# julius-sk/spgemm-gnn

Measured on AMD Instinct MI355X. Metric: SpGEMM+SSpMM edges/sec on Reddit, hidden=256, k in {8,16,32,64}; %HBM roofline, higher is better.
Workload: dtype f32

## Files before the change

spgemm-gnn_amd/csrc/common.h:

```cpp
#pragma once

#include <hip/hip_runtime.h>
#include <stdint.h>

#include <string>
#include <vector>

#include "device_buf.h"
#include "maxk_hip.h"

namespace maxk {

constexpr int kWave = 64;
constexpr int kFwdTileRows = 32;
constexpr int kFwdMaxTileRows = 64;
constexpr int kFwdRowPad = 1;
constexpr int kFwdColBits = 26;
constexpr uint32_t kFwdColMask = (1u << kFwdColBits) - 1;
constexpr int kFwdThreads = 256;
constexpr int kBwdThreads = 512;
constexpr int kMaxDim = 256;
constexpr int kFwdUnroll = 8;
constexpr int kFwdFlagChunk3 = 1;
constexpr int kFwdFlagQuad = 2;
constexpr int kFwdFlagChunk2 = 4;
constexpr int kBwdTasksPerCu = 2;
constexpr int kBwdMinTaskEdges = 100000;
constexpr int kXcds = 8;
constexpr int kFwdRotWindows = 16;
constexpr double kFwdSlotEdgeRate = 1.6e8;
constexpr double kFwdSlotEdgeRateFixed = 3.0e8;
constexpr double kFwdPackedTableBytes = 150e6;
constexpr double kFwdPackedTableBytes16 = 32e6;
constexpr long long kFwdPackMinEdgesPerCol = 40;
constexpr long long kFwdPackMinEdgesPerColL2 = 128;
constexpr double kFwdSelL2Bytes = 3e6;
constexpr double kBwdTwoPassReuse = 0.75;
constexpr int kBwdRowsPerWave = 4;
constexpr double kBwdTwoPassWorkspaceCap = 16.0 * (1ull << 30);
constexpr int kStatsBlocksPerCu = 4;
constexpr int kBwdRecPad = 16 * kWave + kWave;
constexpr int kBwdLdsBudget = 160 * 1024;

void set_error(const std::string& msg);

#define MAXK_CHECK_ARG(cond, msg)                 \
  do {                                            \
    if (!(cond)) {                                \
      ::maxk::set_error(msg);                     \
      return MAXK_ERR_INVALID_ARG;                \
    }                                             \
  } while (0)

#define MAXK_HIP_TRY(expr)                                                      \
  do {                                                                          \
    hipError_t _e = (expr);                                                     \
    if (_e != hipSuccess) {                                                     \
      ::maxk::set_error(std::string(#expr) + ": " + hipGetErrorString(_e));     \
      return (int)_e;                                                           \
    }                                                                           \
  } while (0)

#define MAXK_LAUNCH_CHECK(what)                                                 \
  do {                                                                          \
    hipError_t _e = hipGetLastError();                                          \
    if (_e != hipSuccess) {                                                     \
      ::maxk::set_error(std::string(what) + ": " + hipGetErrorString(_e));      \
      return (int)_e;                                                           \
    }                                                                           \
  } while (0)

inline bool ranges_overlap(const void* a, int64_t na, const void* b, int64_t nb) {
  const uintptr_t x = reinterpret_cast<uintptr_t>(a), y = reinterpret_cast<uintptr_t>(b);
  return na > 0 && nb > 0 && x < y + (uintptr_t)nb && y < x + (uintptr_t)na;
}

struct FwdTask {
  int32_t row0;
  int32_t nrows;
  int32_t e0;
  int32_t e1;
};
static_assert(sizeof(FwdTask) == 16, "FwdTask is loaded as one dwordx4");

inline int cbsr_record_bytes(int k) {
  const int b = 5 * k;
  return b <= 64 ? 64 : b <= 128 ? 128 : (b + 15) / 16 * 16;
}

// ... 21 lines not shown
struct BwdTask {
  int32_t col0;
  int32_t ncols;
  int32_t e0;
  int32_t e1;
  int32_t shared;
  int32_t group;
  int32_t chunk;
  int32_t slab;
};
static_assert(sizeof(BwdTask) == 32, "BwdTask is 2 x dwordx4");


__device__ __forceinline__ void lds_add(double* p, double v) {
  __hip_atomic_fetch_add(p, v, __ATOMIC_RELAXED, __HIP_MEMORY_SCOPE_WORKGROUP);
}

__device__ __forceinline__ void global_add(float* p, float v) {
  __hip_atomic_fetch_add(p, v, __ATOMIC_RELAXED, __HIP_MEMORY_SCOPE_AGENT);
}

}

struct maxk_plan {
  int32_t num_nodes = 0;
  int32_t num_cols = 0;
  int64_t num_edges = 0;
  int32_t dim_origin = 0;
  int32_t dim_k = 0;
  const int32_t* src_ptr = nullptr;
  const int32_t* src_idx = nullptr;
  int32_t cus = 256;
  int32_t fwd_tile_rows = 32;
  int32_t fwd_waves = 4;
  int32_t fwd_unroll = 8;
  int32_t fwd_rec_bytes = 0;
  maxk::DeviceBuf<uint8_t> fwd_rec;
  int32_t fwd_fixed = 0;
  maxk::DeviceBuf<int2> fwd_fix;
  maxk::DeviceBuf<int32_t> fwd_rowptr;
  int64_t fwd_xstat_off = 0;
  maxk::DeviceBuf<maxk::FwdTask> fwd_tasks;
  int32_t fwd_phases = 1;
  int32_t fwd_rot_ticks = 0;
  int32_t fwd_chunk3 = 0;
  int32_t fwd_chunk2 = 0;
  int32_t fwd_quad = 0;
  int32_t fwd_two_tables = 0;
  maxk::DeviceBuf<int32_t> fwd_phase_off;
  maxk::DeviceBuf<int32_t> fwd_perm;
  maxk::DeviceBuf<uint2> fwd_cv;
  int32_t fwd_rowconst = 0;
  int32_t fwd_rowconst_off = 0;
  maxk::DeviceBuf<uint32_t> fwd_cv4;
  maxk::DeviceBuf<float> fwd_rowval;
  int32_t n_fwd_tasks = 0;
  maxk::DeviceBuf<int32_t> zero_rows;
  int32_t n_zero_rows = 0;
  int32_t bwd_feats = 4;
  int32_t bwd_slot_groups = 1;
  int32_t bwd_kp = 0;
  int32_t bwd_ks = 0;
  int32_t bwd_unroll = 8;
  int32_t bwd_waves = 8;
  int32_t bwd_big = 0;
  int32_t bwd_block_cols = 0;
  int32_t n_bwd_blocks = 0;
  maxk::DeviceBuf<maxk::BwdTask> bwd_tasks;
  int32_t n_bwd_tasks = 0;
  int32_t n_bwd_shared = 0;
  maxk::DeviceBuf<int32_t> bwd_perm;
  maxk::DeviceBuf<uint32_t> bwd_rec;
  maxk::DeviceBuf<uint32_t> bwd_sel;
  int32_t bwd_twopass = 0;
  int32_t bwd_tp_rows = 1;
  maxk::DeviceBuf<uint32_t> bwd_erec;
  maxk::DeviceBuf<float> bwd_tbuf;
  maxk::DeviceBuf<int32_t> bwd_colptr;
  int32_t bwd_tp_chunks = 1;
  std::vector<int32_t> tp_rows;
  std::vector<int64_t> tp_edges;
  maxk::DeviceBuf<int32_t> bwd_colptr2;
  int32_t col_order = 1;
  maxk::DeviceBuf<int32_t> bwd_corder;
  int64_t bwd_slab_floats = 0;
  int64_t bwd_slab_off = 0;
  maxk::DeviceBuf<int4> bwd_combine;
  int32_t n_bwd_combine = 0;
  int64_t device_bytes = 0;
  int32_t external_ws = 0;
  int64_t fwd_ws_bytes = 0;
  int64_t bwd_ws_bytes = 0;
  int32_t bwd_row_order = 1;
  int32_t fwd_handout = 1;
  int32_t bwd_handout = 1;
};

inline bool plan_fwd_rowconst_shape(const maxk_plan* p) {
  const int k = p->dim_k;
  if (!(k % 4 == 0 || p->fwd_chunk3 || p->fwd_chunk2)) return false;
  const int Lf = p->fwd_chunk3 ? (k + 2) / 3 : p->fwd_chunk2 ? k / 2 : k / 4;
  return p->fwd_quad && Lf % 4 == 0 && p->fwd_unroll == 8 && p->fwd_fix;
}

inline int plan_fwd_layout(const maxk_plan* p) {
  if (p->fwd_chunk2) return 4;
  if (p->fwd_chunk3) return 2;
  if (p->dim_k % 4 != 0) return 3;
  return p->fwd_two_tables ? 0 : 1;
}
```

spgemm-gnn_amd/csrc/plan.hip:

```cpp
#include <hipcub/hipcub.hpp>

#include <algorithm>
#include <cmath>
#include <cstddef>
#include <cstring>
#include <memory>
#include <utility>
#include <vector>

#include "common.h"

namespace maxk {


__global__ void expand_rows_kernel(const int32_t* __restrict__ ptr, int N,
                                   int32_t* __restrict__ row_of) {
  const int lane = threadIdx.x & (kWave - 1);
  const int row = blockIdx.x * (256 / kWave) + threadIdx.x / kWave;
  if (row >= N) return;
  const int e1 = ptr[row + 1];
  for (int e = ptr[row] + lane; e < e1; e += kWave) row_of[e] = row;
}

__global__ void fwd_key_kernel(const int32_t* __restrict__ idx, const int32_t* __restrict__ row_of,
// ... 571 lines not shown
                 "maxk_plan_create: fwd_chunk3 must be 0, 1, 2 or 3");
  MAXK_CHECK_REMOVED(o.bwd_cas64 == 0 || o.bwd_cas64 == 1, "bwd_cas64 = 2");
  MAXK_CHECK_REMOVED(o.quad_loads == 0, "quad_loads");
  MAXK_CHECK_ARG(o.fwd_two_tables >= 0 && o.fwd_two_tables <= 2,
                 "maxk_plan_create: fwd_two_tables must be 0, 1 or 2");
  MAXK_CHECK_ARG(o.external_workspace == 0 || o.external_workspace == 1,
                 "maxk_plan_create: external_workspace must be 0 or 1");
  MAXK_CHECK_ARG(o.bwd_flush >= 0 && o.bwd_flush <= 2,
                 "maxk_plan_create: bwd_flush must be 0, 1 or 2");
  MAXK_CHECK_ARG(o.bwd_chunk_bounds >= 0 && o.bwd_chunk_bounds <= 3,
                 "maxk_plan_create: bwd_chunk_bounds must be 0 or 2");
  MAXK_CHECK_REMOVED(o.bwd_chunk_bounds == 0 || o.bwd_chunk_bounds == 2,
                     "bwd_chunk_bounds 1 (shared rows) / 3 (equal cost)");
  MAXK_CHECK_ARG(o.fwd_fixed >= 0 && o.fwd_fixed <= 2,
                 "maxk_plan_create: fwd_fixed must be 0, 1 or 2");
  MAXK_CHECK_ARG(o.bwd_tp_store >= 0 && o.bwd_tp_store <= 2,
                 "maxk_plan_create: bwd_tp_store must be 0 or 1");
  MAXK_CHECK_REMOVED(o.bwd_tp_store != 2, "bwd_tp_store = 2 (column-order products)");
  MAXK_CHECK_REMOVED(o.bwd_row_cost == 0, "bwd_row_cost");
  MAXK_CHECK_ARG(o.col_order >= 0 && o.col_order <= 4,
                 "maxk_plan_create: col_order must be 0, 1, 2 or 4");
  MAXK_CHECK_REMOVED(o.col_order != 3, "col_order = 3 (clustered)");
  MAXK_CHECK_ARG(o.bwd_row_order >= 0 && o.bwd_row_order <= 2,
                 "maxk_plan_create: bwd_row_order must be 0, 1 or 2");
  MAXK_CHECK_ARG(o.fwd_rowconst >= 0 && o.fwd_rowconst <= 2,
                 "maxk_plan_create: fwd_rowconst must be 0, 1 or 2");
  return MAXK_OK;
}

static int device_cus() {
  int dev = 0;
  hipDeviceProp_t prop;
  if (hipGetDevice(&dev) == hipSuccess && hipGetDeviceProperties(&prop, dev) == hipSuccess &&
      prop.multiProcessorCount > 0)
    return prop.multiProcessorCount;
  return 256;
}

namespace {

struct PlanBuild {
  const int32_t* ptr;
  const int32_t* idx;
  const float* val;
  int32_t N, NC;
  int64_t E;
  int32_t D, k;
  const maxk_plan_options& o;
  const int32_t* user_order;
  hipStream_t s;
  std::vector<int32_t> hp;
  std::unique_ptr<maxk_plan> plan;
  bool big_table = false;
  int C = 1, S = 1;
  int order_mode = 1;
  bool twopass = false;
  bool row_hash_ok = false, row_hash = false;
  int64_t ra = 1, rb = 0;
  int rbits = 1;
  int nblocks = 0;
  const int32_t* bcolpos = nullptr;
  std::vector<FwdTask> ftasks;
  std::vector<int32_t> zrows;
  std::vector<int64_t> offs;
  std::vector<BwdTask> btasks;
  int nshared = 0;
  DeviceBuf<int32_t> row_of;
  DeviceBuf<int32_t> order;
  DeviceBuf<int32_t> colpos;
  DeviceBuf<uint32_t> bkeys;
  DeviceBuf<int32_t> brow;
  DeviceBuf<int32_t> bcol;
};

}

static int hip_fail(const char* what, hipError_t e) {
  set_error(std::string("maxk_plan_create: ") + what + ": " + hipGetErrorString(e));
  return (int)e;
}
#define PLAN_TRY(expr)                                         \
  do {                                                         \
    const hipError_t _e = (expr);                              \
    if (_e != hipSuccess) return hip_fail(#expr, _e);          \
  } while (0)

static int check_args(const PlanBuild& ctx) {
  const maxk_plan_options& o = ctx.o;
  const int32_t N = ctx.N, NC = ctx.NC, D = ctx.D, k = ctx.k;
  const int64_t E = ctx.E;
  const int32_t *ptr = ctx.ptr, *idx = ctx.idx, *user_order = ctx.user_order;
  if (const int rc = check_options(o)) return rc;
  MAXK_CHECK_ARG(o.col_order != 4 || user_order != nullptr || NC == 0,
                 "maxk_plan_create: col_order 4 needs the col_order argument");
  MAXK_CHECK_ARG(NC >= 0 && (E == 0 || NC > 0), "maxk_plan_create: num_cols out of range");
  if ((uint32_t)NC > kFwdColMask + 1u) {
    set_error("maxk_plan_create: more than 2^26 source columns is not supported");
    return MAXK_ERR_UNSUPPORTED;
  }
  MAXK_CHECK_ARG(N >= 0 && E >= 0 && E < (int64_t)INT32_MAX,
                 "maxk_plan_create: sizes out of range (E must fit int32)");
  MAXK_CHECK_ARG(D >= 1 && D <= kMaxDim, "maxk_plan_create: dim_origin must be in [1, 256]");
  MAXK_CHECK_ARG(k >= 1 && k <= D, "k must be between 1 and input dimension");
  MAXK_CHECK_ARG(ptr != nullptr && (E == 0 || idx != nullptr), "maxk_plan_create: null pointer");
  return MAXK_OK;
}

static void choose_fwd_shape(PlanBuild& ctx) {
  maxk_plan* p = ctx.plan.get();
  const maxk_plan_options& o = ctx.o;
  const int32_t N = ctx.N, NC = ctx.NC, D = ctx.D, k = ctx.k;
  const int cus = p->cus;
  const int fwd_row_bytes = (D + kFwdRowPad) * 8;
  const int fwd_two_wg_rows = std::min(kFwdMaxTileRows, (kBwdLdsBudget / 2 - 256) / fwd_row_bytes);
  const bool fwd_lds_two_wg = 3 * kFwdTileRows * fwd_row_bytes > kBwdLdsBudget &&
                              (int64_t)N >= (int64_t)fwd_two_wg_rows * 10 * cus;
  p->fwd_tile_rows = o.fwd_tile_rows ? o.fwd_tile_rows
                     : fwd_lds_two_wg ? fwd_two_wg_rows : kFwdTileRows;
  const int waves_rec = o.fwd_waves ? o.fwd_waves : (k == 16 && o.fwd_unroll != 4 ? 4 : 8);
  p->fwd_chunk2 = (o.fwd_chunk3 == 3 || (o.fwd_chunk3 == 0 && k == 16)) && k % 2 == 0 &&
                  k / 2 <= kWave;
  p->fwd_waves = p->fwd_chunk2 && !o.fwd_waves ? 8 : waves_rec;
  p->fwd_unroll = o.fwd_unroll ? o.fwd_unroll : (p->fwd_waves == 8 && k == 48 ? 4 : 8);
  p->fwd_chunk3 = (o.fwd_chunk3 == 1 ||
                   ((o.fwd_chunk3 == 0 || (o.fwd_chunk3 == 3 && !p->fwd_chunk2)) && k % 16 != 0)) &&
                  (k + 2) / 3 <= kWave;
  ctx.big_table = (double)std::max(NC, 1) * 5.0 * k >
                (k >= 32 ? kFwdPackedTableBytes : kFwdPackedTableBytes16);
  p->fwd_fixed = (o.fwd_fixed == 1 || (o.fwd_fixed == 0 && k >= 16 && !ctx.big_table)) &&
                 (k % 4 == 0 || p->fwd_chunk3 || p->fwd_chunk2);
  p->fwd_quad = p->fwd_fixed;
}

static void choose_bwd_shape(PlanBuild& ctx) {
  maxk_plan* p = ctx.plan.get();
  const maxk_plan_options& o = ctx.o;
  const int32_t N = ctx.N, NC = ctx.NC, D = ctx.D, k = ctx.k;
  const int64_t E = ctx.E;
  const int lds_budget = o.bwd_lds_bytes ? o.bwd_lds_bytes : kBwdLdsBudget;
  bool two_slots = false;
  if (k == 8 && N > 0 && NC > 0) {
    const double c0 = std::min<double>(NC, (lds_budget - 16) / (5.0 * k));
    two_slots = (double)E / N * c0 / NC < 10.0;
  }
  int F = o.bwd_features_per_lane ? o.bwd_features_per_lane
                                  : (two_slots || (k % 4 == 2 && k <= 2 * kWave) ? 2 : 4);
  if (F == 2 && (k + 1) / 2 > kWave) F = 4;
  p->bwd_feats = F;
  const int kF = (k + F - 1) / F * F;
  int S = o.bwd_slot_groups ? o.bwd_slot_groups : 1;
  if (o.bwd_slot_groups == 0 && F == 4 && k >= 16 && k % 8 == 0 && N > 0 && NC > 0) {
    const double c1 = std::min<double>(NC, (lds_budget - 16) / (5.0 * k));
    if ((double)E / N * c1 / NC < 4.5) S = 2;
  }
  while (S > 1 && kF % (F * S) != 0) S >>= 1;
  if (o.bwd_features_per_lane == 0 && F == 4 && S == 2 && kF / S == 8) {
    F = 2;
    p->bwd_feats = F;
  }
  p->bwd_slot_groups = S;
  p->bwd_kp = kF;
  p->bwd_ks = kF / S;
  p->bwd_unroll = o.bwd_unroll ? o.bwd_unroll : (F == 2 ? 12 : 8);
  p->bwd_waves = o.bwd_waves ? o.bwd_waves : (k >= 32 ? 12 : 8);
  p->bwd_big = (uint64_t)N * (uint64_t)D * 4u > 0xffffffffull;
  int C = std::max(1, (lds_budget - 16) / (5 * p->bwd_ks));
  C = std::min(C, std::max(NC, 1));
  ctx.C = C;
  ctx.S = S;
}

static hipError_t need_row_of(PlanBuild& ctx) {
  if (ctx.row_of || ctx.E == 0) return hipSuccess;
  const hipError_t e = ctx.row_of.alloc((size_t)ctx.E);
  if (e != hipSuccess) return e;
  hipLaunchKernelGGL(expand_rows_kernel, dim3((ctx.N + 3) / 4), dim3(256), 0, ctx.s, ctx.ptr,
                     ctx.N, ctx.row_of);
  return hipGetLastError();
}

static int read_ptr(PlanBuild& ctx) {
  const int32_t N = ctx.N;
// ... 75 lines not shown
    PLAN_TRY(hipGetLastError());
    PLAN_TRY(sort_pairs(d_tmp, d_kin, d_kout, d_ids, p->fwd_perm, E, cbits + tbits, s));
    PLAN_TRY(plan_alloc(p, p->fwd_cv, (size_t)E + 1, true));
    PLAN_TRY(hipMemsetAsync(p->fwd_cv + E, 0, sizeof(uint2), s));
    hipLaunchKernelGGL(gather_fwd_kernel, dim3(grid_for(E, 256)), dim3(256), 0, s,
                       p->fwd_perm, ctx.idx, d_rl, ctx.val, E, p->fwd_cv, true);
    PLAN_TRY(hipGetLastError());
    PLAN_TRY(hipStreamSynchronize(s));
  }
  return MAXK_OK;
}

static int build_forward(PlanBuild& ctx) {
  maxk_plan* p = ctx.plan.get();
  const maxk_plan_options& o = ctx.o;
  std::vector<FwdTask>& ftasks = ctx.ftasks;
  std::vector<int32_t>& zrows = ctx.zrows;
  const int32_t N = ctx.N, NC = ctx.NC, k = ctx.k;
  const int64_t E = ctx.E;
  hipStream_t s = ctx.s;
  build_fwd_tasks(ctx.hp, N, p->fwd_tile_rows, o.fwd_task_cap, ftasks, zrows);
  p->n_fwd_tasks = (int32_t)ftasks.size();
  p->n_zero_rows = (int32_t)zrows.size();
  if (!ftasks.empty()) {
    const int nt = (int)ftasks.size();
    if (const int rc = sort_fwd_edges(ctx)) return rc;
    PLAN_TRY(plan_alloc(p, p->fwd_tasks, ftasks.size()));
    PLAN_TRY(upload(p->fwd_tasks, ftasks, s));
    if (p->fwd_fixed) {
      PLAN_TRY(plan_alloc(p, p->fwd_fix, ftasks.size()));
      PLAN_TRY(plan_alloc(p, p->fwd_rowptr, (size_t)N + 1));
      PLAN_TRY(hipMemcpyAsync(p->fwd_rowptr, ctx.ptr, sizeof(int32_t) * ((size_t)N + 1),
                              hipMemcpyDeviceToDevice, s));
      PLAN_TRY(fwd_fix_stats(p, p->fwd_rowptr, ctx.val, s));
    }
    int B = 1;
    p->fwd_rot_ticks = 0;
    const bool low_reuse = o.fwd_rotate == 0 && NC > 0 && (double)E / NC < 64.0;
    if (o.fwd_rotate != 2 && !low_reuse && (k % 4 == 0 || p->fwd_chunk3 || p->fwd_chunk2)) {
      const int Bd = p->fwd_fixed ? (k >= 64 ? 64 : k >= 32 ? 32 : kFwdRotWindows) : kFwdRotWindows;
      B = o.fwd_rot_windows > 0 ? std::min(o.fwd_rot_windows, 64) : Bd;
      const double rate = o.fwd_rot_rate > 0 ? o.fwd_rot_rate * 1e6
                                             : std::min(5e8, std::max(2e7, (p->fwd_fixed ? kFwdSlotEdgeRateFixed : kFwdSlotEdgeRate) * 16.0 / k));
      const double tile_ticks = (double)E / nt / rate * 1e8;
      p->fwd_rot_ticks = (int)std::max(1.0, tile_ticks / B);
    }
    B = std::max(1, std::min(B, std::max(NC, 1)));
    p->fwd_phases = B;
    PLAN_TRY(plan_alloc(p, p->fwd_phase_off, (size_t)nt * (B + 1)));
    hipLaunchKernelGGL(fwd_phase_kernel, dim3((nt * (B + 1) + 255) / 256), dim3(256), 0, s,
                       p->fwd_tasks, nt, p->fwd_cv, NC, B, p->fwd_phase_off);
    PLAN_TRY(hipGetLastError());
    p->fwd_rowconst_off = o.fwd_rowconst == 2;
    PLAN_TRY(fwd_set_values(p, p->fwd_rowptr, ctx.val, true, s));
  }
  if (!zrows.empty()) {
    PLAN_TRY(plan_alloc(p, p->zero_rows, zrows.size()));
    PLAN_TRY(upload(p->zero_rows, zrows, s));
  }
  return MAXK_OK;
}

static int layout_fwd_workspace(PlanBuild& ctx) {
  maxk_plan* p = ctx.plan.get();
  const maxk_plan_options& o = ctx.o;
  const int32_t NC = ctx.NC, k = ctx.k;
  const int64_t E = ctx.E;
  const bool big_table = ctx.big_table;
  const bool sel_l2 = (double)std::max(NC, 1) * k <= kFwdSelL2Bytes;
  const bool few_edges = E < kFwdPackMinEdgesPerCol * std::max(NC, 1) ||
                         (sel_l2 && E < kFwdPackMinEdgesPerColL2 * std::max(NC, 1));
  p->fwd_two_tables = !p->fwd_chunk3 && !p->fwd_chunk2 && k % 4 == 0 &&
                      (o.fwd_two_tables == 1 ||
                       (o.fwd_two_tables == 0 &&
                        (k >= 64 || (!big_table && (k >= 32 || few_edges)))));
  if (p->fwd_two_tables) {
  } else if ((p->fwd_chunk3 || p->fwd_chunk2) && NC > 0) {
    const int b = (p->fwd_chunk3 ? (k + 2) / 3 : k / 2) * 16;
    p->fwd_rec_bytes = b <= 64 ? 64 : b <= 128 ? 128 : b;
    p->fwd_ws_bytes = (int64_t)NC * p->fwd_rec_bytes;
  } else if (k % 4 == 0 && NC > 0) {
    p->fwd_rec_bytes = cbsr_record_bytes(k);
    p->fwd_ws_bytes = (int64_t)NC * p->fwd_rec_bytes;
  }
  if (p->fwd_fix) {
    p->fwd_xstat_off = (p->fwd_ws_bytes + 255) / 256 * 256;
    p->fwd_ws_bytes = p->fwd_xstat_off + 256;
  }
  if (p->fwd_ws_bytes > 0 && !p->external_ws)
    PLAN_TRY(plan_alloc(p, p->fwd_rec, (size_t)p->fwd_ws_bytes));
  return MAXK_OK;
}

static void choose_bwd_algo(PlanBuild& ctx) {
  maxk_plan* p = ctx.plan.get();
  const maxk_plan_options& o = ctx.o;
  const std::vector<int32_t>& hp = ctx.hp;
  const int32_t N = ctx.N, NC = ctx.NC, k = ctx.k;
  const int64_t E = ctx.E;
  int C = ctx.C;
  const int Lt = k / 4;
  int R = 1;
  while (R < kBwdRowsPerWave && (double)R * E / std::max(N, 1) < 256.0) R *= 2;
  bool tp_fits = true;
  for (int r0 = 0; r0 < N && tp_fits; r0 += R)
    tp_fits = (uint64_t)(hp[std::min(N, r0 + R)] - hp[r0]) * (uint64_t)k * 4u < 0x80000000ull;
// ... 378 lines not shown
    p->bwd_waves = 8;
    p->bwd_unroll = 8;
  }
}

static int upload_backward(PlanBuild& ctx) {
  maxk_plan* p = ctx.plan.get();
  const int64_t E = ctx.E;
  hipStream_t s = ctx.s;
  if (!ctx.btasks.empty()) {
    PLAN_TRY(plan_alloc(p, p->bwd_tasks, ctx.btasks.size()));
    PLAN_TRY(upload(p->bwd_tasks, ctx.btasks, s));
  }
  if (!ctx.twopass && E > 0) {
    PLAN_TRY(plan_alloc(p, p->bwd_rec, 3 * (size_t)(E + kBwdRecPad), true));
    PLAN_TRY(hipMemsetAsync(p->bwd_rec + 3 * E, 0, sizeof(uint32_t) * 3 * kBwdRecPad, s));
    hipLaunchKernelGGL(build_bwd_rec_kernel, dim3(grid_for(E, 256)), dim3(256), 0, s,
                       p->bwd_perm, ctx.brow, ctx.bcol, ctx.val, E, ctx.C, ctx.D,
                       p->bwd_big, p->bwd_rec);
    PLAN_TRY(hipGetLastError());
    p->bwd_slab_off = 0;
    p->bwd_ws_bytes = p->bwd_slab_floats * 4;
    if (!p->external_ws && p->bwd_ws_bytes > 0)
      PLAN_TRY(plan_alloc(p, p->bwd_sel, (size_t)p->bwd_slab_floats));
  }
  PLAN_TRY(hipStreamSynchronize(s));
  p->col_order = 1;
  if (ctx.order && ctx.bcolpos) {
    p->col_order = ctx.order_mode;
    plan_adopt(p, p->bwd_corder, std::move(ctx.order));
  }
  return MAXK_OK;
}
#undef PLAN_TRY

static int plan_create_impl(const int32_t* ptr, const int32_t* idx, const float* val, int32_t N,
                            int32_t NC, int64_t E, int32_t D, int32_t k,
                            const maxk_plan_options& o, const int32_t* user_order, void* stream,
                            maxk_plan** out_plan) {
  *out_plan = nullptr;
  PlanBuild ctx{ptr, idx, val, N, NC, E, D, k, o, user_order, (hipStream_t)stream};
  if (const int rc = check_args(ctx)) return rc;
  ctx.plan.reset(new maxk_plan());
  maxk_plan* p = ctx.plan.get();
  p->external_ws = o.external_workspace;
  p->num_nodes = N;
  p->num_cols = NC;
  p->num_edges = E;
  p->dim_origin = D;
  p->dim_k = k;
  p->src_ptr = ptr;
  p->src_idx = idx;
  p->cus = device_cus();
  choose_fwd_shape(ctx);
  choose_bwd_shape(ctx);
  int rc = read_ptr(ctx);
  if (rc == MAXK_OK) rc = build_column_order(ctx);
  if (rc == MAXK_OK) rc = build_forward(ctx);
  if (rc == MAXK_OK) rc = layout_fwd_workspace(ctx);
  if (rc == MAXK_OK) {
    choose_bwd_algo(ctx);
    rc = sort_bwd_blocks(ctx);
  }
  if (rc == MAXK_OK && E > 0) rc = ctx.twopass ? build_two_pass(ctx) : gather_block_edges(ctx);
  if (rc == MAXK_OK && !ctx.twopass && E > 0 && ctx.nblocks > 0) rc = emit_block_tasks(ctx);
  if (rc != MAXK_OK) return rc;
  deal_to_xcds(ctx);
  resolve_launch_shape(ctx);
  if (const int rc2 = upload_backward(ctx)) return rc2;
  *out_plan = ctx.plan.release();
  return MAXK_OK;
}

extern "C" int maxk_plan_refresh_values(maxk_plan* p, const float* val, void* stream) {
  MAXK_CHECK_ARG(p != nullptr, "maxk_plan_refresh_values: plan is null");
  if (p->num_edges == 0) return MAXK_OK;
  hipStream_t s = (hipStream_t)stream;
  const int g = grid_for(p->num_edges, 256);
  if (p->bwd_erec)
    hipLaunchKernelGGL(build_erec_kernel, dim3(g), dim3(256), 0, s, nullptr, nullptr, 1, val,
                       p->num_edges, p->bwd_erec);
  else if (p->bwd_rec)
    hipLaunchKernelGGL(build_bwd_rec_kernel, dim3(g), dim3(256), 0, s, p->bwd_perm, nullptr,
                       nullptr, val, p->num_edges, p->bwd_block_cols, p->dim_origin, p->bwd_big,
                       p->bwd_rec);
  {
    const hipError_t e = fwd_set_values(p, p->fwd_rowptr, val, false, s);
    if (e != hipSuccess) {
      set_error(std::string("maxk_plan_refresh_values: ") + hipGetErrorString(e));
      return (int)e;
    }
  }
  MAXK_LAUNCH_CHECK("maxk_plan_refresh_values launch");
  return MAXK_OK;
}

extern "C" int maxk_plan_fwd_rowconst(const maxk_plan* p, int32_t* rowconst) {
  MAXK_CHECK_ARG(p != nullptr && rowconst != nullptr, "maxk_plan_fwd_rowconst: null pointer");
  *rowconst = p->fwd_rowconst;
  return MAXK_OK;
}

extern "C" int maxk_plan_get_info(const maxk_plan* p, maxk_plan_info* info) {
  return maxk_plan_get_info_sized(p, info, (int64_t)offsetof(maxk_plan_info, col_order));
}

extern "C" int maxk_plan_get_info_sized(const maxk_plan* p, maxk_plan_info* out,
                                        int64_t info_bytes) {
  MAXK_CHECK_ARG(p != nullptr && out != nullptr && info_bytes >= 0,
// ... 63 lines not shown
```

spgemm-gnn_amd/csrc/spgemm.hip:

```cpp
#include <algorithm>
#include <type_traits>

#include "common.h"

namespace maxk {

template <int W>
__device__ __forceinline__ uint32_t quad_bcast(uint32_t v) {
  static_assert(W >= 0 && W < 4, "quad lane");
  return (uint32_t)__builtin_amdgcn_update_dpp(0, (int)v, W * 0x55, 0xf, 0xf, false);
}

__device__ __forceinline__ uint32_t quad_pick(uint32_t v, int u) {
  switch (u & 3) {
    case 0: return quad_bcast<0>(v);
    case 1: return quad_bcast<1>(v);
    case 2: return quad_bcast<2>(v);
    default: return quad_bcast<3>(v);
  }
}

struct LdsF64 {
  using T = double;
  using V = float;
// ... 168 lines not shown
    mn = min(mn, lo);
  }
  for (int o = kWave / 2; o > 0; o >>= 1) {
    mx = max(mx, (uint32_t)__shfl_xor((int)mx, o));
    mn = min(mn, (uint32_t)__shfl_xor((int)mn, o));
  }
  const int w = threadIdx.x / kWave;
  if ((threadIdx.x & (kWave - 1)) == 0) { smx[w] = mx; smn[w] = mn; }
  __syncthreads();
  if (threadIdx.x == 0) {
    for (int i = 1; i < 256 / kWave; ++i) { mx = max(mx, smx[i]); mn = min(mn, smn[i]); }
    atomicMax(st0, mx);
    atomicMax(st1, 0x7fffffffu - mn);
  }
}


template <int V>
__global__ void pack_cbsr3_kernel(const float* __restrict__ sp_data,
                                  const uint8_t* __restrict__ sp_index,
                                  uint8_t* __restrict__ rec, int ncols, int k, int rec_bytes,
                                  int ds, int is) {
  const int chunks = (k + V - 1) / V;
  const int64_t total = (int64_t)ncols * chunks;
  for (int64_t t = (int64_t)blockIdx.x * blockDim.x + threadIdx.x; t < total;
       t += (int64_t)gridDim.x * blockDim.x) {
    const int64_t c = t / chunks;
    const int j = (int)(t - c * chunks);
    uint32_t w[4] = {0u, 0u, 0u, 0u};
#pragma unroll
    for (int i = 0; i < V; ++i) {
      const int l = V * j + i;
      if (l < k) {
        w[i] = __float_as_uint(sp_data[c * ds + l]);
        w[V == 3 ? 3 : 2] |= (uint32_t)sp_index[c * is + l] << (8 * i);
      }
    }
    *reinterpret_cast<uint4*>(rec + c * rec_bytes + j * 16) = make_uint4(w[0], w[1], w[2], w[3]);
  }
}

template <class A, int FL, int U, bool RC>
__device__ __forceinline__ void fwd_edges4(typename A::T* acc, int e0, int e1, int* ctr,
                                           int wave, int nwaves, int EPS, int slot, int l0,
                                           bool lane_on,
                                           const void* __restrict__ cvp,
                                           const uint8_t* __restrict__ rec, int rec_bytes,
                                           const uint8_t* __restrict__ seltab, int ss, int D,
                                           int k, double sc, const float* __restrict__ rowval) {
  using T = typename A::T;
  constexpr bool C3 = (FL & kFwdFlagChunk3) != 0;
  constexpr bool C2 = (FL & kFwdFlagChunk2) != 0;
  constexpr bool EM = (FL & kFwdFlagQuad) != 0;
  static_assert(!RC || (EM && U == 8), "4-byte edge words: quad windows of 8 sub-steps");
  const uint2* cv = static_cast<const uint2*>(cvp);
  const int last = e1 - 1;
  const int qq = threadIdx.x & 3;
  for (int i = 0;; ++i) {
    int wi = wave + i * nwaves;
    if (ctr) {
      int c = 0;
      if ((threadIdx.x & (kWave - 1)) == 0) c = atomicAdd(ctr, 1);
      wi = __builtin_amdgcn_readlane(c, 0);
    }
    const int base = (EM && U == 8 ? (e0 & ~1) : e0) + wi * (EPS * U);
    if (base >= e1) break;
    uint32_t cw[U];
    float v[U];
    bool ok[U];
    if constexpr (RC) {
      const int sb = base + slot * U;
      const uint2 wq =
          *reinterpret_cast<const uint2*>(static_cast<const uint32_t*>(cvp) + min(sb + 2 * qq, last & ~1));
#pragma unroll
      for (int u = 0; u < U; ++u) {
        const uint32_t w0 = quad_pick((u & 1) ? wq.y : wq.x, u >> 1);
        ok[u] = lane_on && sb + u >= e0 && sb + u < e1;
        cw[u] = ok[u] ? w0 : (w0 & kFwdColMask);
        if constexpr (A::kFixed) v[u] = 1.0f;
        else v[u] = rowval[cw[u] >> kFwdColBits];
      }
    } else if constexpr (EM && U == 8) {
      const int sb = base + slot * U;
      const uint4 wq = *reinterpret_cast<const uint4*>(cv + min(sb + 2 * qq, last & ~1));
#pragma unroll
      for (int u = 0; u < U; ++u) {
        const uint32_t w0 = quad_pick((u & 1) ? wq.z : wq.x, u >> 1);
        const uint32_t w1 = quad_pick((u & 1) ? wq.w : wq.y, u >> 1);
        ok[u] = lane_on && sb + u >= e0 && sb + u < e1;
        cw[u] = ok[u] ? w0 : (w0 & kFwdColMask);
        v[u] = __uint_as_float(w1);
      }
    } else if constexpr (EM) {
      uint2 wq[U / 4];
#pragma unroll
      for (int j = 0; j < U / 4; ++j) wq[j] = cv[min(base + slot * U + 4 * j + qq, last)];
#pragma unroll
      for (int u = 0; u < U; ++u) {
        ok[u] = lane_on && base + slot * U + u < e1;
        cw[u] = quad_pick(wq[u / 4].x, u);
        v[u] = __uint_as_float(quad_pick(wq[u / 4].y, u));
      }
    } else {
#pragma unroll
      for (int u = 0; u < U; ++u) {
        const int e = base + u * EPS + slot;
        ok[u] = lane_on && e < e1;
        const uint2 w = cv[ok[u] ? e : last];
        cw[u] = w.x;
        v[u] = __uint_as_float(w.y);
      }
    }
    float4 x[U];
    uint32_t sel[U];
#pragma unroll
    for (int u = 0; u < U; ++u) {
      const uint8_t* rp = rec + (size_t)(cw[u] & kFwdColMask) * rec_bytes;
      if constexpr (C3) {
        const uint4 w = *reinterpret_cast<const uint4*>(rp + l0 * 16);
        x[u] = make_float4(__uint_as_float(w.x), __uint_as_float(w.y), __uint_as_float(w.z), 0.f);
        sel[u] = w.w;
      } else if constexpr (C2) {
        const uint4 w = *reinterpret_cast<const uint4*>(rp + l0 * 16);
        x[u] = make_float4(__uint_as_float(w.x), __uint_as_float(w.y), 0.f, 0.f);
        sel[u] = w.z;
      } else {
        x[u] = *reinterpret_cast<const float4*>(rp + l0 * 4);
        const uint8_t* sp = seltab ? seltab + (size_t)(cw[u] & kFwdColMask) * ss + l0
                                   : rp + 4 * k + l0;
        sel[u] = *reinterpret_cast<const uint32_t*>(sp);
      }
    }
    if constexpr (!A::kFixed) {
#pragma unroll
      for (int u = 0; u < U; ++u)
        if (!ok[u]) x[u] = make_float4(0.f, 0.f, 0.f, 0.f);
    }
#pragma unroll
    for (int u = 0; u < U; ++u) {
      T* arow = acc + (cw[u] >> kFwdColBits) * D;
      const uint32_t sv = sel[u];
      const typename A::V vu = A::scale(ok[u] ? v[u] : 0.f, sc);
      if constexpr (C3) {
        A::add2(arow + (sv & 0xffu), vu, x[u].x);
// ... 66 lines not shown
  constexpr bool C3 = (FL & kFwdFlagChunk3) != 0;
  constexpr bool C2 = (FL & kFwdFlagChunk2) != 0;
  const int L = (VEC == 4) ? (C3 ? (k + 2) / 3 : C2 ? k / 2 : k / 4) : (k < kWave ? k : kWave);
  const int EPS = kWave / L;
  const int lane = threadIdx.x & (kWave - 1);
  const int wave = threadIdx.x / kWave;
  const int slot = lane / L;
  const int l0 = (lane - slot * L) * (C3 || C2 ? 1 : VEC);
  const bool lane_on = slot < EPS;
  constexpr int kWaves = NT / kWave;

  if constexpr (VEC == 4) {
    auto sweep = [&](auto* a, auto tag) {
      using AA = decltype(tag);
      int* c0 = handout ? &s_win[0] : nullptr;
      int* c1 = handout ? &s_win[1] : nullptr;
      if (emid >= 0) {
        fwd_edges4<AA, FL, FU, RC>(a, emid, t.e1, c0, wave, kWaves, EPS, slot, l0, lane_on, cv, rec,
                           rec_bytes, seltab, ss, DS, k, fsc, RC ? rowval + t.row0 : nullptr);
        fwd_edges4<AA, FL, FU, RC>(a, t.e0, emid, c1, wave, kWaves, EPS, slot, l0, lane_on, cv, rec,
                           rec_bytes, seltab, ss, DS, k, fsc, RC ? rowval + t.row0 : nullptr);
      } else {
        fwd_edges4<AA, FL, FU, RC>(a, t.e0, t.e1, c0, wave, kWaves, EPS, slot, l0, lane_on, cv, rec,
                           rec_bytes, seltab, ss, DS, k, fsc, RC ? rowval + t.row0 : nullptr);
      }
    };
    if (fixed) sweep(acc64, LdsFix{});
    else sweep(acc, LdsF64{});
  } else {
    for (int base = t.e0 + wave * EPS; base < t.e1; base += kWaves * EPS) {
      const int e = base + slot;
      if (lane_on && e < t.e1) {
        const uint2 w = static_cast<const uint2*>(cv)[e];
        const float v = __uint_as_float(w.y);
        double* arow = acc + (w.x >> kFwdColBits) * DS;
        const size_t c = w.x & kFwdColMask;
        for (int l = l0; l < k; l += L)
          LdsF64::add2(arow + sp_index[c * ss + l], v, sp_data[c * ds + l]);
      }
    }
  }
  __syncthreads();

  float* dst = out + (size_t)t.row0 * D;
  const double finv = fixed ? 1.0 / fsc : 0.0;
  auto rowscale = [&](int r) -> double {
    if constexpr (RC) return (double)rowval[t.row0 + r];
    return 1.0;
  };
  auto get = [&](int i, double rs) -> float {
    const int r = i / D;
    double a = fixed ? fwd_fix_decode(acc64[r * DS + (i - r * D)], finv) : acc[r * DS + (i - r * D)];
    if constexpr (RC) {
      if (fixed) a *= rs;
    }
    return (float)a;
  };
  if (!split) {
    const bool add = accum && fixed;
    if ((D & 3) == 0) {
      for (int i = threadIdx.x * 4; i < n; i += NT * 4) {
        const double rs = rowscale(i / D);
        float4 v = make_float4(get(i, rs), get(i + 1, rs), get(i + 2, rs), get(i + 3, rs));
        if (add) {
          const float4 o = *reinterpret_cast<const float4*>(dst + i);
          v = make_float4(o.x + v.x, o.y + v.y, o.z + v.z, o.w + v.w);
        }
        *reinterpret_cast<float4*>(dst + i) = v;
      }
    } else {
      for (int i = threadIdx.x; i < n; i += NT) {
        const float a = get(i, rowscale(i / D));
        dst[i] = add ? dst[i] + a : a;
      }
    }
  } else {
    const double rs = rowscale(0);
    for (int i = threadIdx.x; i < D; i += NT) global_add(dst + i, get(i, rs));
  }
}

__global__ void zero_rows_kernel(const int32_t* __restrict__ rows, int nrows, float* out,
                                 int D) {
  const int r = blockIdx.x;
  if (r >= nrows) return;
  float* dst = out + (size_t)rows[r] * D;
  for (int i = threadIdx.x; i < D; i += blockDim.x) dst[i] = 0.f;
}

template <int N, int F>
__device__ __forceinline__ void bwd_cas_update(unsigned* accq, int KS, const uint32_t (&cl)[N],
                                               const float (&x)[N][F], const bool (&ok)[N]) {
  using u64 = unsigned long long;
  u64 old2[N][F / 2];
#pragma unroll
  for (int u = 0; u < N; ++u) {
    if constexpr (F == 4) {
      const uint4 o4 = *reinterpret_cast<const uint4*>(accq + cl[u] * KS);
      old2[u][0] = (u64)o4.x | ((u64)o4.y << 32);
      old2[u][1] = (u64)o4.z | ((u64)o4.w << 32);
    } else {
      const uint2 o2 = *reinterpret_cast<const uint2*>(accq + cl[u] * KS);
      old2[u][0] = (u64)o2.x | ((u64)o2.y << 32);
    }
  }
  auto addp = [](u64 o, float a0, float a1) -> u64 {
    const float lo = __uint_as_float((unsigned)o) + a0;
// ... 501 lines not shown
  MAXK_LAUNCH_CHECK("cbsr_stats launch");
  return MAXK_OK;
}

static int check_plan(const maxk_plan* plan, const int32_t* ptr, const int32_t* idx,
                      int32_t N, int64_t E, int32_t k, int32_t D, const char* who) {
  MAXK_CHECK_ARG(plan != nullptr, std::string(who) + ": plan is null");
  if (plan->num_nodes != N || plan->num_edges != E || plan->dim_k != k ||
      plan->dim_origin != D || plan->src_ptr != ptr || plan->src_idx != idx) {
    set_error(std::string(who) + ": plan was built for a different graph / k / D");
    return MAXK_ERR_PLAN_MISMATCH;
  }
  return MAXK_OK;
}

static int table_strides(int64_t& ds, int64_t& is, int k, const char* who) {
  if (ds == 0) ds = k;
  if (is == 0) is = k;
  MAXK_CHECK_ARG(ds >= k && is >= k && ds <= INT32_MAX / 4 && is <= INT32_MAX,
                 std::string(who) + ": table row strides must be >= k (0: k)");
  return MAXK_OK;
}

static int launch_spgemm_fwd(const maxk_plan* plan, const float* sp_data, int ds,
                             const uint8_t* sp_index, int is, const uint8_t* recp, int rec_bytes,
                             const uint8_t* seltab, float* out, int D, int k, int accum,
                             const int2* fix_tab, const uint32_t* xstat, int xs_n, int xs_stride,
                             int xs_off2, size_t lds, hipStream_t s) {
  const bool pairs = plan->fwd_chunk2;
  if (plan->n_fwd_tasks == 0) return MAXK_OK;
  const int Lf = plan->fwd_chunk3 ? (k + 2) / 3 : pairs ? k / 2 : k / 4;
  const int FL = (plan->fwd_chunk3 ? kFwdFlagChunk3 : 0) | (pairs ? kFwdFlagChunk2 : 0) |
                 (plan->fwd_quad && Lf % 4 == 0 ? kFwdFlagQuad : 0);
  const int fwaves = plan->fwd_waves;
  const bool rc = plan->fwd_rowconst != 0;
  if (rc && !plan_fwd_rowconst_shape(plan)) {
    set_error("spgemm_fwd launch: 4-byte edge words on a plan whose kernel has none");
    return MAXK_ERR_UNSUPPORTED;
  }
  const void* cvp = rc ? static_cast<const void*>(plan->fwd_cv4.get())
                       : static_cast<const void*>(plan->fwd_cv.get());
#define FWD_LAUNCH_NT(V, FF, NT, FU, RC)                                                    \
  do {                                                                                      \
    if (lds > 64 * 1024) MAXK_HIP_TRY(allow_lds(spgemm_fwd_kernel<V, FF, NT, FU, RC>, lds)); \
    hipLaunchKernelGGL((spgemm_fwd_kernel<V, FF, NT, FU, RC>), dim3(plan->n_fwd_tasks),     \
                       dim3(NT), lds, s, plan->fwd_tasks, plan->fwd_phase_off,              \
                       plan->fwd_phases, cvp, sp_data, sp_index, recp, rec_bytes, out, D, k, \
                       plan->fwd_rot_ticks, seltab, is, ds, accum, fix_tab, xstat, xs_n,     \
                       xs_stride, xs_off2, plan->fwd_handout == 2 ? 1 : 0,                  \
                       plan->fwd_rowval.get());                                             \
  } while (0)
#define FWD_LAUNCH(V, FF, RCOK)  \
  do {                                                                                      \
    if (rc && fwaves == 8) FWD_LAUNCH_NT(V, FF, 8 * kWave, kFwdUnroll, RCOK);               \
    else if (rc) FWD_LAUNCH_NT(V, FF, kFwdThreads, kFwdUnroll, RCOK);                       \
    else if (fwaves == 8 && plan->fwd_unroll == 4) FWD_LAUNCH_NT(V, FF, 8 * kWave, 4, false); \
    else if (fwaves == 8) FWD_LAUNCH_NT(V, FF, 8 * kWave, kFwdUnroll, false);               \
    else FWD_LAUNCH_NT(V, FF, kFwdThreads, kFwdUnroll, false);                              \
  } while (0)
  if (k % 4 == 0 || plan->fwd_chunk3 || plan->fwd_chunk2) {
    switch (FL) {
      case 0: FWD_LAUNCH(4, 0, false); break;
      case kFwdFlagChunk3: FWD_LAUNCH(4, kFwdFlagChunk3, false); break;
      case kFwdFlagQuad: FWD_LAUNCH(4, kFwdFlagQuad, true); break;
      case kFwdFlagChunk2: FWD_LAUNCH(4, kFwdFlagChunk2, false); break;
      case kFwdFlagChunk2 | kFwdFlagQuad: FWD_LAUNCH(4, kFwdFlagChunk2 | kFwdFlagQuad, true); break;
      default: FWD_LAUNCH(4, kFwdFlagChunk3 | kFwdFlagQuad, true); break;
    }
  } else {
    FWD_LAUNCH(1, 0, false);
  }
#undef FWD_LAUNCH
#undef FWD_LAUNCH_NT
  MAXK_LAUNCH_CHECK("spgemm_fwd launch");
  return MAXK_OK;
}

static int spgemm_forward_impl(const maxk_plan* plan, const int32_t* ptr, const int32_t* idx,
                               const float* val, const float* sp_data, int64_t ds64,
                               const uint8_t* sp_index, int64_t is64, float* out, int32_t N,
                               int64_t E, int32_t k, int32_t D, void* stream, int accum,
                               void* ws, int64_t ws_bytes, const uint32_t* stats = nullptr,
                               int n_stats = 0, int64_t stats_stride = 2) {
  MAXK_CHECK_ARG(N >= 0 && E >= 0, "maxk_spgemm_forward: negative size");
  MAXK_CHECK_ARG(stats == nullptr || (n_stats >= 1 && n_stats <= 1024),
                 "maxk_spgemm_forward_ex: n_stats must be in [1, 1024]");
  if (stats_stride == 0) stats_stride = 2;
  MAXK_CHECK_ARG(stats_stride >= 2 && stats_stride * (int64_t)n_stats < (int64_t)INT32_MAX,
                 "maxk_spgemm_forward_ex: stats_stride must be >= 2 (or 0)");
  MAXK_CHECK_ARG(D >= 1 && D <= kMaxDim, "maxk_spgemm_forward: dim_origin must be in [1, 256]");
  MAXK_CHECK_ARG(k >= 1 && k <= D, "k must be between 1 and input dimension");
  if (int rc = table_strides(ds64, is64, k, "maxk_spgemm_forward")) return rc;
  const int ds = (int)ds64, is = (int)is64;
  int rc = check_plan(plan, ptr, idx, N, E, k, D, "maxk_spgemm_forward");
  if (rc) return rc;
  if (N == 0) return MAXK_OK;
  MAXK_CHECK_ARG(out && sp_data && sp_index && (E == 0 || (idx && val)) && ptr,
                 "maxk_spgemm_forward: null pointer");
  (void)val;
  uint8_t* ws_base = plan->fwd_rec;
  if (ws) {
    MAXK_CHECK_ARG(ws_bytes >= plan->fwd_ws_bytes,
                   "maxk_spgemm_forward: workspace smaller than maxk_plan_workspace_bytes");
    ws_base = static_cast<uint8_t*>(ws);
  } else if (plan->fwd_ws_bytes > 0 && !ws_base) {
    set_error("maxk_spgemm_forward: the plan has an external workspace; use maxk_spgemm_forward_ws");
    return MAXK_ERR_INVALID_ARG;
// ... 349 lines not shown
```

Measured before the change: 100.2 billion.

## Enable row-constant chunk2 fixed-point forward path for k=8 on large graphs

Adds a plan-time probe that checks whether each row's values are constant. For k=8 on large graphs without big tables, it then selects the chunk2 (pairs) layout with fixed-point accumulation and 4-byte edge words. It also adds a 4-sub-step unroll variant of the row-constant edge loader and a matching launch path. The aim is to cut per-edge memory traffic (4-byte instead of 8-byte column/value words) and use the quad fixed-point accumulation for k=8. The cost is an extra probe kernel plus a host sync during planning, and more kernel variants.

```diff
diff --git a/spgemm-gnn_amd/csrc/common.h b/spgemm-gnn_amd/csrc/common.h
--- a/spgemm-gnn_amd/csrc/common.h
+++ b/spgemm-gnn_amd/csrc/common.h
@@ -35,6 +35,7 @@
 constexpr long long kFwdPackMinEdgesPerCol = 40;
 constexpr long long kFwdPackMinEdgesPerColL2 = 128;
 constexpr double kFwdSelL2Bytes = 3e6;
+constexpr long long kFwdRowconstPairsMinEdges = 1ll << 24;
 constexpr double kBwdTwoPassReuse = 0.75;
 constexpr int kBwdRowsPerWave = 4;
 constexpr double kBwdTwoPassWorkspaceCap = 16.0 * (1ull << 30);
@@ -162,6 +163,7 @@
   maxk::DeviceBuf<uint2> fwd_cv;
   int32_t fwd_rowconst = 0;
   int32_t fwd_rowconst_off = 0;
+  int32_t fwd_rowconst_on = 0;
   maxk::DeviceBuf<uint32_t> fwd_cv4;
   maxk::DeviceBuf<float> fwd_rowval;
   int32_t n_fwd_tasks = 0;
@@ -210,7 +212,9 @@
   const int k = p->dim_k;
   if (!(k % 4 == 0 || p->fwd_chunk3 || p->fwd_chunk2)) return false;
   const int Lf = p->fwd_chunk3 ? (k + 2) / 3 : p->fwd_chunk2 ? k / 2 : k / 4;
-  return p->fwd_quad && Lf % 4 == 0 && p->fwd_unroll == 8 && p->fwd_fix;
+  const bool windows = p->fwd_unroll == 8 ||
+                       (p->fwd_rowconst_on && p->fwd_unroll == 4 && p->fwd_waves == 8);
+  return p->fwd_quad && Lf % 4 == 0 && windows && p->fwd_fix;
 }
 
 inline int plan_fwd_layout(const maxk_plan* p) {
diff --git a/spgemm-gnn_amd/csrc/plan.hip b/spgemm-gnn_amd/csrc/plan.hip
--- a/spgemm-gnn_amd/csrc/plan.hip
+++ b/spgemm-gnn_amd/csrc/plan.hip
@@ -647,6 +647,7 @@
   std::vector<int32_t> hp;
   std::unique_ptr<maxk_plan> plan;
   bool big_table = false;
+  bool rc_pairs = false;
   int C = 1, S = 1;
   int order_mode = 1;
   bool twopass = false;
@@ -701,6 +702,29 @@
   return MAXK_OK;
 }
 
+static int probe_rowconst_pairs(PlanBuild& ctx) {
+  const maxk_plan_options& o = ctx.o;
+  const bool big_table = (double)std::max(ctx.NC, 1) * 5.0 * ctx.k > kFwdPackedTableBytes16;
+  if (ctx.k != 8 || o.fwd_chunk3 || o.fwd_fixed || o.fwd_rowconst == 2 || o.fwd_unroll == 4 ||
+      big_table || ctx.N <= 0 || ctx.E == 0 ||
+      (o.fwd_rowconst != 1 && ctx.E < kFwdRowconstPairsMinEdges))
+    return MAXK_OK;
+  hipStream_t s = ctx.s;
+  DeviceBuf<float> rv;
+  DeviceBuf<int> d_bad;
+  int bad = 1;
+  PLAN_TRY(rv.alloc((size_t)ctx.N));
+  PLAN_TRY(d_bad.alloc(1));
+  PLAN_TRY(hipMemsetAsync(d_bad, 0, sizeof(int), s));
+  hipLaunchKernelGGL(fwd_rowconst_kernel, dim3((ctx.N + 3) / 4), dim3(256), 0, s, ctx.ptr, ctx.val,
+                     ctx.N, rv, d_bad);
+  PLAN_TRY(hipGetLastError());
+  PLAN_TRY(hipMemcpyAsync(&bad, d_bad, sizeof(int), hipMemcpyDeviceToHost, s));
+  PLAN_TRY(hipStreamSynchronize(s));
+  ctx.rc_pairs = bad == 0;
+  return MAXK_OK;
+}
+
 static void choose_fwd_shape(PlanBuild& ctx) {
   maxk_plan* p = ctx.plan.get();
   const maxk_plan_options& o = ctx.o;
@@ -713,16 +737,17 @@
   p->fwd_tile_rows = o.fwd_tile_rows ? o.fwd_tile_rows
                      : fwd_lds_two_wg ? fwd_two_wg_rows : kFwdTileRows;
   const int waves_rec = o.fwd_waves ? o.fwd_waves : (k == 16 && o.fwd_unroll != 4 ? 4 : 8);
-  p->fwd_chunk2 = (o.fwd_chunk3 == 3 || (o.fwd_chunk3 == 0 && k == 16)) && k % 2 == 0 &&
-                  k / 2 <= kWave;
+  p->fwd_chunk2 = (o.fwd_chunk3 == 3 || (o.fwd_chunk3 == 0 && (k == 16 || ctx.rc_pairs))) &&
+                  k % 2 == 0 && k / 2 <= kWave;
   p->fwd_waves = p->fwd_chunk2 && !o.fwd_waves ? 8 : waves_rec;
   p->fwd_unroll = o.fwd_unroll ? o.fwd_unroll : (p->fwd_waves == 8 && k == 48 ? 4 : 8);
   p->fwd_chunk3 = (o.fwd_chunk3 == 1 ||
-                   ((o.fwd_chunk3 == 0 || (o.fwd_chunk3 == 3 && !p->fwd_chunk2)) && k % 16 != 0)) &&
+                   ((o.fwd_chunk3 == 0 || o.fwd_chunk3 == 3) && !p->fwd_chunk2 && k % 16 != 0)) &&
                   (k + 2) / 3 <= kWave;
   ctx.big_table = (double)std::max(NC, 1) * 5.0 * k >
                 (k >= 32 ? kFwdPackedTableBytes : kFwdPackedTableBytes16);
-  p->fwd_fixed = (o.fwd_fixed == 1 || (o.fwd_fixed == 0 && k >= 16 && !ctx.big_table)) &&
+  p->fwd_fixed = (o.fwd_fixed == 1 ||
+                  (o.fwd_fixed == 0 && (k >= 16 || ctx.rc_pairs) && !ctx.big_table)) &&
                  (k % 4 == 0 || p->fwd_chunk3 || p->fwd_chunk2);
   p->fwd_quad = p->fwd_fixed;
 }
@@ -904,6 +929,7 @@
                        p->fwd_tasks, nt, p->fwd_cv, NC, B, p->fwd_phase_off);
     PLAN_TRY(hipGetLastError());
     p->fwd_rowconst_off = o.fwd_rowconst == 2;
+    p->fwd_rowconst_on = o.fwd_rowconst == 1;
     PLAN_TRY(fwd_set_values(p, p->fwd_rowptr, ctx.val, true, s));
   }
   if (!zrows.empty()) {
@@ -1388,9 +1414,11 @@
   p->src_ptr = ptr;
   p->src_idx = idx;
   p->cus = device_cus();
+  int rc = probe_rowconst_pairs(ctx);
+  if (rc != MAXK_OK) return rc;
   choose_fwd_shape(ctx);
   choose_bwd_shape(ctx);
-  int rc = read_ptr(ctx);
+  rc = read_ptr(ctx);
   if (rc == MAXK_OK) rc = build_column_order(ctx);
   if (rc == MAXK_OK) rc = build_forward(ctx);
   if (rc == MAXK_OK) rc = layout_fwd_workspace(ctx);
diff --git a/spgemm-gnn_amd/csrc/spgemm.hip b/spgemm-gnn_amd/csrc/spgemm.hip
--- a/spgemm-gnn_amd/csrc/spgemm.hip
+++ b/spgemm-gnn_amd/csrc/spgemm.hip
@@ -244,7 +244,8 @@
   constexpr bool C3 = (FL & kFwdFlagChunk3) != 0;
   constexpr bool C2 = (FL & kFwdFlagChunk2) != 0;
   constexpr bool EM = (FL & kFwdFlagQuad) != 0;
-  static_assert(!RC || (EM && U == 8), "4-byte edge words: quad windows of 8 sub-steps");
+  static_assert(!RC || (EM && (U == 8 || U == 4)),
+                "4-byte edge words: quad windows of 8 or 4 sub-steps");
   const uint2* cv = static_cast<const uint2*>(cvp);
   const int last = e1 - 1;
   const int qq = threadIdx.x & 3;
@@ -260,7 +261,7 @@
     uint32_t cw[U];
     float v[U];
     bool ok[U];
-    if constexpr (RC) {
+    if constexpr (RC && U == 8) {
       const int sb = base + slot * U;
       const uint2 wq =
           *reinterpret_cast<const uint2*>(static_cast<const uint32_t*>(cvp) + min(sb + 2 * qq, last & ~1));
@@ -282,6 +283,18 @@
         ok[u] = lane_on && sb + u >= e0 && sb + u < e1;
         cw[u] = ok[u] ? w0 : (w0 & kFwdColMask);
         v[u] = __uint_as_float(w1);
+      }
+    } else if constexpr (RC) {
+      const uint32_t* cv4 = static_cast<const uint32_t*>(cvp);
+      uint32_t wq[U / 4];
+#pragma unroll
+      for (int j = 0; j < U / 4; ++j) wq[j] = cv4[min(base + slot * U + 4 * j + qq, last)];
+#pragma unroll
+      for (int u = 0; u < U; ++u) {
+        ok[u] = lane_on && base + slot * U + u < e1;
+        cw[u] = quad_pick(wq[u / 4], u);
+        if constexpr (A::kFixed) v[u] = 1.0f;
+        else v[u] = rowval[cw[u] >> kFwdColBits];
       }
     } else if constexpr (EM) {
       uint2 wq[U / 4];
@@ -454,7 +467,7 @@
     const int r = i / D;
     double a = fixed ? fwd_fix_decode(acc64[r * DS + (i - r * D)], finv) : acc[r * DS + (i - r * D)];
     if constexpr (RC) {
-      if (fixed) a *= rs;
+      if (fixed) a = a * rs + 0.0;
     }
     return (float)a;
   };
@@ -1062,7 +1075,8 @@
   } while (0)
 #define FWD_LAUNCH(V, FF, RCOK)  \
   do {                                                                                      \
-    if (rc && fwaves == 8) FWD_LAUNCH_NT(V, FF, 8 * kWave, kFwdUnroll, RCOK);               \
+    if (rc && fwaves == 8 && plan->fwd_unroll == 4) FWD_LAUNCH_NT(V, FF, 8 * kWave, 4, RCOK); \
+    else if (rc && fwaves == 8) FWD_LAUNCH_NT(V, FF, 8 * kWave, kFwdUnroll, RCOK);          \
     else if (rc) FWD_LAUNCH_NT(V, FF, kFwdThreads, kFwdUnroll, RCOK);                       \
     else if (fwaves == 8 && plan->fwd_unroll == 4) FWD_LAUNCH_NT(V, FF, 8 * kWave, 4, false); \
     else if (fwaves == 8) FWD_LAUNCH_NT(V, FF, 8 * kWave, kFwdUnroll, false);               \
```

Result: no change. 100.5 billion (median of 4 runs) (+0.3%).
